# aurelienpierreeng/ansel

Measured on AMD Instinct MI355X. Metric: MPix/s full export pixelpipe (100 MP raw); % MI355X HBM roofline, higher is better.
Workload: dtype f32

## Files before the change

### ansel_amd/csrc/diffuse.hip

```cpp
#include "hip_common.h"

#include <type_traits>
#include "devmath.h"
#include "ieee_inrange.h"
#include "px_colorspaces.h"

#include <math.h>
#include <cstdlib>

namespace ansel
{
int bspline_launch_decompose(int devid, hipStream_t s, const float4 *in, float4 *hf, float4 *lf, int w, int h, int mult,
                             const unsigned *gate = nullptr);
int bspline_launch_decompose3(int devid, hipStream_t s, const void *in, bool in4, float *lf, int w, int h, int mult, unsigned *alpha_flag);
#ifdef ANSEL_HIP_MEASURING
int bspline_launch_decompose2(int devid, hipStream_t s, const float4 *in, float4 *low1, float4 *low2, int w, int h, int mult);
#endif
}
using namespace ansel;

namespace
{

#define DIFFUSE_MAX_SCALES 10
#define BSPLINE_SIGMA 1.0553651328015339f
#define PDE_KAPPA 0.25f

__device__ __forceinline__ float max_first(const float a, const float b) { return a > b ? a : b; }
__device__ __forceinline__ float max_zero(const float v) { return isfinite(v) ? max_first(v, 0.0f) : 0.0f; }
__device__ __forceinline__ int clampi(const int v, const int lo, const int hi) { return v < lo ? lo : (v > hi ? hi : v); }

__device__ __forceinline__ int walk_row(const int b, const int height, const int mult)
{
  if(height <= mult) return b < height ? b : -1;
  const int per_pass = (height + mult - 1) / mult;
  const int row = (b % per_pass) * mult + b / per_pass;
  return row < height ? row : -1;
}

struct pde_args
{
  int width, height, mult;
  float anisotropy[4];
  int kind[4];
  int same02, same13;
  float variance_threshold, regularization;
  float abcd[4], strength;
  int wskip;
  int post_lab;
  float post_m[3][4];
  int approx_div;
  int off;
  const unsigned *gate;
  int gate_sense;
};

#ifdef ANSEL_HIP_MEASURING
#define PDE_APPROX(a) ((a).approx_div != 0)
#define PDE_OFF(a, bit) (((a).off & (bit)) != 0)
#else
#define PDE_APPROX(a) false
#define PDE_OFF(a, bit) false
#endif
__device__ __forceinline__ float div_1ulp(const float x, const float y)
{
  const float r = __builtin_amdgcn_rcpf(y);
  const float q = x * r;
  return __builtin_fmaf(__builtin_fmaf(-y, q, x), r, q);
}

__device__ __forceinline__ float fast_expf(const float x)
{
  const float t = 1065353216.0f + x * 11401300.0f;
  int k = (t > -2147483648.0f && t < 2147483648.0f) ? (int)t : 0;
  k = k > 0 ? k : 0;
  return __int_as_float(k);
}

__device__ __forceinline__ float direction(float gx, float gy, float &cos2, float &sin2, float &cs, const bool approx = false)
{
  const float s2 = gx * gx + gy * gy;
// ... 286 lines not shown

#define PDE_RING 4
#define PDE_DMA_MAX_MULT 16
#if defined(__HIP_DEVICE_COMPILE__) && !defined(__gfx950__)
#error "pde_dma_planes(): LDS-DMA of 16 bytes per lane and its hazard padding are written for gfx950 only"
#endif
template <int NPL>
__device__ __forceinline__ void pde_dma_planes(const float4 *const p0, const float4 *const p1, const float4 *const p2, const unsigned voff,
                                               const unsigned d0, const unsigned d1, const unsigned d2)
{
  unsigned keep;
  if constexpr(NPL == 3)
    asm volatile("s_waitcnt lgkmcnt(0)\n\ts_nop 4\n\ts_mov_b32 %0, m0\n\t"
                 "s_mov_b32 m0, %5\n\ts_nop 0\n\tglobal_load_lds_dwordx4 %1, %2\n\t"
                 "s_mov_b32 m0, %6\n\ts_nop 0\n\tglobal_load_lds_dwordx4 %1, %3\n\t"
                 "s_mov_b32 m0, %7\n\ts_nop 0\n\tglobal_load_lds_dwordx4 %1, %4\n\t"
                 "s_mov_b32 m0, %0"
                 : "=&s"(keep)
                 : "v"(voff), "s"(p0), "s"(p1), "s"(p2), "s"(d0), "s"(d1), "s"(d2)
                 : "memory");
  else
    asm volatile("s_waitcnt lgkmcnt(0)\n\ts_nop 4\n\ts_mov_b32 %0, m0\n\t"
                 "s_mov_b32 m0, %4\n\ts_nop 0\n\tglobal_load_lds_dwordx4 %1, %2\n\t"
                 "s_mov_b32 m0, %5\n\ts_nop 0\n\tglobal_load_lds_dwordx4 %1, %3\n\t"
                 "s_mov_b32 m0, %0"
                 : "=&s"(keep)
                 : "v"(voff), "s"(p0), "s"(p2), "s"(d0), "s"(d2)
                 : "memory");
}
template <bool H0_4>
__device__ __forceinline__ void pde_dma_planes3(const void *const p0, const void *const p1, const void *const p2, const unsigned voff0,
                                                const unsigned voff, const unsigned d0, const unsigned d1, const unsigned d2)
{
  unsigned keep;
  if constexpr(H0_4)
    asm volatile("s_waitcnt lgkmcnt(0)\n\ts_nop 4\n\ts_mov_b32 %0, m0\n\t"
                 "s_mov_b32 m0, %6\n\ts_nop 0\n\tglobal_load_lds_dwordx4 %1, %3\n\t"
                 "s_mov_b32 m0, %7\n\ts_nop 0\n\tglobal_load_lds_dwordx3 %2, %4\n\t"
                 "s_mov_b32 m0, %8\n\ts_nop 0\n\tglobal_load_lds_dwordx3 %2, %5\n\t"
                 "s_mov_b32 m0, %0"
                 : "=&s"(keep)
                 : "v"(voff0), "v"(voff), "s"(p0), "s"(p1), "s"(p2), "s"(d0), "s"(d1), "s"(d2)
                 : "memory");
  else
    asm volatile("s_waitcnt lgkmcnt(0)\n\ts_nop 4\n\ts_mov_b32 %0, m0\n\t"
                 "s_mov_b32 m0, %5\n\ts_nop 0\n\tglobal_load_lds_dwordx3 %1, %2\n\t"
                 "s_mov_b32 m0, %6\n\ts_nop 0\n\tglobal_load_lds_dwordx3 %1, %3\n\t"
                 "s_mov_b32 m0, %7\n\ts_nop 0\n\tglobal_load_lds_dwordx3 %1, %4\n\t"
                 "s_mov_b32 m0, %0"
                 : "=&s"(keep)
                 : "v"(voff), "s"(p0), "s"(p1), "s"(p2), "s"(d0), "s"(d1), "s"(d2)
                 : "memory");
}
struct pde_px3
{
  float x, y, z;
};
template <bool HSUB, int MODE, bool DMA, int L3>
__device__ __forceinline__ void pde_strip_body(const float4 *__restrict__ hf, const float4 *__restrict__ hsub,
                                               const float4 *__restrict__ lf, float4 *__restrict__ out, const pde_args &a,
                                               const int final_pass, const unsigned char *__restrict__ mask, const int strip,
                                               const int strips_per_class)
{
  static_assert(L3 == 0 || (HSUB && DMA), "three-float planes: the low-pass chain's LDS-DMA form only");
  if(a.gate && ((*a.gate != 0u) == (a.gate_sense == 1))) return;
  extern __shared__ float4 r2s[];
  pde_px3 *const r2s3 = reinterpret_cast<pde_px3 *>(r2s);
  const int mult = a.mult;
  const int cls = blockIdx.y / strips_per_class, k0s = (blockIdx.y - cls * strips_per_class) * strip;
  const int n_cls = (a.height - cls + mult - 1) / mult;
  if(k0s >= n_cls) return;
  const int nrows = (strip < n_cls - k0s) ? strip : n_cls - k0s;
  const int r_first = cls + k0s * mult;
  const int tx = threadIdx.x, tw = 256 + 2 * mult;
  const int col = (int)blockIdx.x * 256 + tx;
  const bool live = col < a.width;
  const int cols[3] = { clampi(col - mult, 0, a.width - 1), clampi(col, 0, a.width - 1), clampi(col + mult, 0, a.width - 1) };
#define PDE_ROW(v) ((size_t)clampi(r_first + ((v) - 1) * mult, 0, a.height - 1) * a.width)
  float4 Hw[3][3], Lw[3][3];
  constexpr int NPL = HSUB ? 3 : 2;
  const int lane = tx & 63, zw = 64 + 2 * mult;
  float4 *const zone = r2s + PDE_RING * tw + (tx >> 6) * NPL * zw;
  float4 *const zone3 = reinterpret_cast<float4 *>(reinterpret_cast<char *>(r2s) + (size_t)PDE_RING * tw * 12) + (tx >> 6) * 3 * zw;
  using lds_f4_ptr = __attribute__((address_space(3))) float4 *;
  const unsigned zone_lds = !DMA ? 0u : (unsigned)__builtin_amdgcn_readfirstlane((int)(unsigned)(__UINTPTR_TYPE__)(lds_f4_ptr)(
                                           L3 ? zone3 : zone));
  const unsigned off_main = (unsigned)cols[0] * 16u, off_halo = (unsigned)clampi(col - mult + 64, 0, a.width - 1) * 16u;
  auto dma_row = [&](const int v) {
    const size_t y = PDE_ROW(v);
    if constexpr(L3 != 0)
    {
      const unsigned m3 = (unsigned)cols[0] * 12u, h3 = (unsigned)clampi(col - mult + 64, 0, a.width - 1) * 12u;
      const unsigned p0 = (unsigned)zw * 16u, p1 = 2u * p0;
      const void *const b0 = L3 == 2 ? (const void *)(hf + y) : (const void *)((const float *)hf + 3 * y);
      const void *const b1 = (const float *)hsub + 3 * y, *const b2 = (const float *)lf + 3 * y;
      pde_dma_planes3<L3 == 2>(b0, b1, b2, L3 == 2 ? off_main : m3, m3, zone_lds, zone_lds + p0, zone_lds + p1);
      if(lane < 2 * mult)
        pde_dma_planes3<L3 == 2>(b0, b1, b2, L3 == 2 ? off_halo : h3, h3, zone_lds + 1024u, zone_lds + p0 + 1024u, zone_lds + p1 + 1024u);
      return;
    }
    const unsigned pl = (unsigned)zw * 16u;
    pde_dma_planes<NPL>(hf + y, hsub + y, lf + y, off_main, zone_lds, zone_lds + pl, zone_lds + (NPL - 1) * pl);
    if(lane < 2 * mult)
      pde_dma_planes<NPL>(hf + y, hsub + y, lf + y, off_halo, zone_lds + 1024u, zone_lds + pl + 1024u, zone_lds + (NPL - 1) * pl + 1024u);
  };
  struct
  {
    float4 o;
    size_t idx;
    bool have;
  } pending;
  pending.have = false;
  auto store = [&](const size_t i, const float4 o) {
    if(final_pass) nt_store(out + i, o);
    else if constexpr(L3 != 0)
    {
      float *const p3 = (float *)out + 3 * i;
      p3[0] = o.x;
      p3[1] = o.y;
      p3[2] = o.z;
    }
    else out[i] = o;
  };
  auto fetch_row = [&](const int v, auto slot_tag) {
    constexpr int SL = decltype(slot_tag)::value;
    const size_t y = PDE_ROW(v);
    float4 c[3], low[3];
    if constexpr(DMA)
    {
      asm volatile("s_waitcnt vmcnt(0)" : : : "memory");
      if constexpr(L3 != 0)
      {
#pragma unroll
        for(int jj = 0; jj < 3; jj++)
        {
          const int x = lane + jj * mult;
          const float4 v0 = zone3[x], v1 = zone3[zw + x], v2 = zone3[2 * zw + x];
          c[jj] = make_float4(v0.x, v0.y, v0.z, 0.0f);
          low[jj] = make_float4(v1.x, v1.y, v1.z, 0.0f);
          Lw[SL][jj] = make_float4(v2.x, v2.y, v2.z, 0.0f);
        }
      }
      else
#pragma unroll
      for(int jj = 0; jj < 3; jj++)
      {
        c[jj] = zone[lane + jj * mult];
        if(HSUB) low[jj] = zone[zw + lane + jj * mult];
        Lw[SL][jj] = zone[(NPL - 1) * zw + lane + jj * mult];
      }
    }
    else if(PDE_OFF(a, 2) && v >= 2)
    {
#pragma unroll
      for(int jj = 0; jj < 3; jj++)
      {
        c[jj] = Hw[SL][jj];
        low[jj] = make_float4(0.f, 0.f, 0.f, 0.f);
      }
    }
    else
    {
#pragma unroll
      for(int jj = 0; jj < 3; jj++)
      {
        c[jj] = hf[y + cols[jj]];
        if(HSUB) low[jj] = hsub[y + cols[jj]];
        Lw[SL][jj] = lf[y + cols[jj]];
      }
    }
    __builtin_amdgcn_sched_barrier(0);
#pragma unroll
    for(int jj = 0; jj < 3; jj++)
      Hw[SL][jj] = HSUB ? make_float4(c[jj].x - low[jj].x, c[jj].y - low[jj].y, c[jj].z - low[jj].z, c[jj].w - low[jj].w) : c[jj];
    float4 *const ring = r2s + (v % PDE_RING) * tw;
    auto ratios = [&](const float4 h, const float4 l) {
      const bool blank = a.wskip && __builtin_amdgcn_ballot_w64((__float_as_uint(h.w) | __float_as_uint(l.w)) != 0) == 0ull;
      return ratio2_rgb(h, l, blank ? 0.0f : ratio2(h.w, l.w), PDE_APPROX(a));
    };
    if(PDE_OFF(a, 4)) return;
    if constexpr(L3 != 0)
    {
      pde_px3 *const ring3 = r2s3 + (v % PDE_RING) * tw;
      auto put = [&](const int x, const float4 h, const float4 l) {
        const float4 r = ratio2_rgb(h, l, 0.0f, PDE_APPROX(a));
        ring3[x] = { r.x, r.y, r.z };
      };
      put(tx + mult, Hw[SL][1], Lw[SL][1]);
      if(tx < mult) put(tx, Hw[SL][0], Lw[SL][0]);
      if(tx >= 256 - mult) put(tx + 2 * mult, Hw[SL][2], Lw[SL][2]);
      return;
    }
    ring[tx + mult] = ratios(Hw[SL][1], Lw[SL][1]);
    if(tx < mult) ring[tx] = ratios(Hw[SL][0], Lw[SL][0]);
    if(tx >= 256 - mult) ring[tx + 2 * mult] = ratios(Hw[SL][2], Lw[SL][2]);
  };
  auto row_step = [&](auto t_tag, const int kk) {
    constexpr int T = decltype(t_tag)::value, S0 = T, S1 = (T + 1) % 3, S2 = (T + 2) % 3;
    constexpr bool WIDE_READS = MODE >= 0 && !(((MODE % 3) | ((MODE / 9) % 3)) && (((MODE / 3) % 3) | ((MODE / 27) % 3)));
    fetch_row(kk + 2, std::integral_constant<int, S2>());
    if constexpr(DMA)
    {
      if(pending.have)
      {
        store(pending.idx, pending.o);
        pending.have = false;
      }
      if(kk + 1 < nrows) dma_row(kk + 3);
    }
    if(!PDE_OFF(a, 1)) __syncthreads();
    if(!live) return;
    const float4 H4[9] = { Hw[S0][0], Hw[S0][1], Hw[S0][2], Hw[S1][0], Hw[S1][1], Hw[S1][2], Hw[S2][0], Hw[S2][1], Hw[S2][2] };
    const float4 L4[9] = { Lw[S0][0], Lw[S0][1], Lw[S0][2], Lw[S1][0], Lw[S1][1], Lw[S1][2], Lw[S2][0], Lw[S2][1], Lw[S2][2] };
    const int row = r_first + kk * mult;
    const bool blank = L3 != 0 || alpha_is_blank(H4, L4);
    __builtin_amdgcn_sched_barrier(0);
    if(pending.have && !PDE_OFF(a, 8))
    {
      store(pending.idx, pending.o);
      pending.have = false;
    }
    __builtin_amdgcn_sched_barrier(0);
    float4 energy = make_float4(0.f, 0.f, 0.f, 0.f);
    if(PDE_OFF(a, 4)) energy = make_float4(0.5f, 0.5f, 0.5f, 0.5f);
    else if constexpr(L3 != 0)
#pragma unroll
    for(int ii = 0; ii < 3; ii++)
    {
      const pde_px3 *const ring = r2s3 + ((kk + ii) % PDE_RING) * tw + tx;
#pragma unroll
      for(int jj = 0; jj < 3; jj++)
      {
        const pde_px3 r = ring[jj * mult];
        energy.x += r.x;
        energy.y += r.y;
        energy.z += r.z;
      }
      if(!WIDE_READS || ii >= 1) asm volatile("" : "+v"(energy.x), "+v"(energy.y), "+v"(energy.z) : : "memory");
    }
    else
#pragma unroll
    for(int ii = 0; ii < 3; ii++)
    {
      const float4 *const ring = r2s + ((kk + ii) % PDE_RING) * tw + tx;
#pragma unroll
      for(int jj = 0; jj < 3; jj++)
      {
        const float4 r = ring[jj * mult];
        energy.x += r.x;
        energy.y += r.y;
        energy.z += r.z;
        if(!(blank && a.wskip)) energy.w += r.w;
      }
      if(!WIDE_READS || ii >= 1) asm volatile("" : "+v"(energy.x), "+v"(energy.y), "+v"(energy.z), "+v"(energy.w) : : "memory");
    }
    const size_t idx = (size_t)row * a.width + col;
    float4 o;
    if(L3 == 0 && mask && !mask[idx])
    {
      const float4 h = H4[4], l = L4[4];
      o = make_float4(max_zero(h.x + l.x), max_zero(h.y + l.y), max_zero(h.z + l.z), max_zero(h.w + l.w));
    }
    else if(PDE_OFF(a, 16))
      o = make_float4(H4[4].x + energy.x, L4[4].y + energy.y, H4[0].z + energy.z, L4[8].w);
    else
    {
      float H[9], L[9];
#pragma unroll
      for(int k = 0; k < 9; k++) { H[k] = H4[k].x; L[k] = L4[k].x; }
      o.x = pde_channel<MODE>(H, L, energy.x, a);
#pragma unroll
      for(int k = 0; k < 9; k++) { H[k] = H4[k].y; L[k] = L4[k].y; }
      o.y = pde_channel<MODE>(H, L, energy.y, a);
#pragma unroll
      for(int k = 0; k < 9; k++) { H[k] = H4[k].z; L[k] = L4[k].z; }
      o.z = pde_channel<MODE>(H, L, energy.z, a);
      if(blank)
        o.w = 0.0f;
      else
      {
#pragma unroll
        for(int k = 0; k < 9; k++) { H[k] = H4[k].w; L[k] = L4[k].w; }
        o.w = pde_channel<MODE>(H, L, energy.w, a);
      }
    }
    if(a.post_lab) o = px_rgb_to_lab(o, a.post_m);
    pending.o = o;
    pending.idx = idx;
    pending.have = true;
  };
  if constexpr(DMA) dma_row(0);
  fetch_row(0, std::integral_constant<int, 0>());
  if constexpr(DMA) dma_row(1);
  fetch_row(1, std::integral_constant<int, 1>());
  if constexpr(DMA) dma_row(2);
  for(int kk = 0; kk < nrows; kk += 3)
  {
    row_step(std::integral_constant<int, 0>(), kk);
    if(kk + 1 < nrows) row_step(std::integral_constant<int, 1>(), kk + 1);
    if(kk + 2 < nrows) row_step(std::integral_constant<int, 2>(), kk + 2);
  }
  if constexpr(DMA) asm volatile("s_waitcnt vmcnt(0)" : : : "memory");
  if(pending.have) store(pending.idx, pending.o);
#undef PDE_ROW
}

template <bool HSUB, int MODE, bool DMA = false>
__global__ __launch_bounds__(256, 3) void diffuse_pde_strip(const float4 *__restrict__ hf, const float4 *__restrict__ hsub,
                                                         const float4 *__restrict__ lf,
                                                         float4 *__restrict__ out, const pde_args a, const int final_pass,
                                                         const unsigned char *__restrict__ mask, const int strip,
                                                         const int strips_per_class)
{
  pde_strip_body<HSUB, MODE, DMA, 0>(hf, hsub, lf, out, a, final_pass, mask, strip, strips_per_class);
}
template <int MODE, bool H0_4>
__global__ __launch_bounds__(256, 3) void diffuse_pde_strip3(const float4 *__restrict__ hf, const float4 *__restrict__ hsub,
                                                          const float4 *__restrict__ lf, float4 *__restrict__ out, const pde_args a,
                                                          const int final_pass, const int strip, const int strips_per_class)
{
  pde_strip_body<true, MODE, true, H0_4 ? 2 : 1>(hf, hsub, lf, out, a, final_pass, nullptr, strip, strips_per_class);
}

__device__ __forceinline__ uint32_t splitmix32(const uint64_t seed)
{
  uint64_t result = (seed ^ (seed >> 33)) * 0x62a9d9ed799705f5ull;
  result = (result ^ (result >> 28)) * 0xcb24d0a5c88c35b3ull;
  return (uint32_t)(result >> 32);
}

__device__ __forceinline__ float xoshiro128plus(uint32_t state[4])
{
  const uint32_t result = state[0] + state[3];
  const uint32_t t = state[1] << 9;
  state[2] ^= state[0];
  state[3] ^= state[1];
  state[1] ^= state[2];
  state[0] ^= state[3];
  state[2] ^= t;
  state[3] = (state[3] << 11) | (state[3] >> 21);
  return (float)(result >> 8) * 0x1.0p-24f;
}

__device__ __forceinline__ float gaussian_noise(const float mu, const float sigma, const bool flip, uint32_t state[4])
{
  const float x1 = xoshiro128plus(state);
  const float u1 = x1 > 1.17549435e-38f ? x1 : 1.17549435e-38f;
  const float u2 = xoshiro128plus(state);
  const float angle = (float)(6.283185307179586 * (double)u2);
  const float radius = sqrtf(-2.0f * ansel_math::logf_exact(u1));
  const float noise = flip ? radius * ansel_math::cosf_exact(angle) : radius * ansel_math::sinf_exact(angle);
  return noise * sigma + mu;
}

__global__ __launch_bounds__(256) void diffuse_inpaint(const float4 *__restrict__ in, float4 *__restrict__ out,
                                                       unsigned char *__restrict__ mask, const float threshold,
                                                       const size_t npixels, const size_t width, const size_t first_pixel)
{
  const size_t p = (size_t)blockIdx.x * blockDim.x + threadIdx.x;
  if(p >= npixels) return;
  const float4 v = in[p];
  const bool m = v.x > threshold || v.y > threshold || v.z > threshold;
  mask[p] = m ? 1 : 0;
  float4 o = v;
  if(m)
  {
    const size_t k = 4 * (p + first_pixel);
    const uint32_t i = (uint32_t)(k / width);
    const uint32_t j = (uint32_t)(k - i);
    uint32_t state[4] = { splitmix32((uint32_t)(j + 1)), splitmix32((uint64_t)(uint32_t)(j + 1) * (uint32_t)(i + 3)),
                          splitmix32(1337), splitmix32(666) };
    xoshiro128plus(state);
    xoshiro128plus(state);
    xoshiro128plus(state);
    xoshiro128plus(state);
    const bool flip = (i % 2) || (j % 2);
    o.x = fabsf(gaussian_noise(v.x, v.x, flip, state));
    o.y = fabsf(gaussian_noise(v.y, v.y, flip, state));
    o.z = fabsf(gaussian_noise(v.z, v.z, flip, state));
    o.w = fabsf(gaussian_noise(v.w, v.w, flip, state));
  }
  out[p] = o;
}

inline float sqf(const float x) { return x * x; }

float sigma_at_step(const float sigma, const unsigned s)
{
  float acc = sigma;
  for(unsigned k = 1; k <= s; k++) acc = sqrtf(sqf(acc) + sqf(exp2f((float)k) * sigma));
  return acc;
}

unsigned steps_to_sigma(const float sigma_filter, const float sigma_final)
{
  unsigned s = 0;
  float radius = sigma_filter;
  while(radius < sigma_final)
  {
    ++s;
    radius = sqrtf(sqf(radius) + sqf((float)(1 << s) * sigma_filter));
  }
  return s + 1;
}

int scales_of(const dt_hip_piece_t *piece, const dt_hip_diffuse_data_t *d)
{
  const float zoom = (float)(d->iscale / piece->roi_in.scale);
  const float final_radius = (float)(d->radius + d->radius_center) * 2.0f / zoom;
  const int s = (int)steps_to_sigma(BSPLINE_SIGMA, final_radius);
  return s < 1 ? 1 : (s > DIFFUSE_MAX_SCALES ? DIFFUSE_MAX_SCALES : s);
}

}

namespace ansel
{
int diffuse_halo_rows(const dt_hip_piece_t *piece, const dt_hip_diffuse_data_t *d)
{
  if(!(d->iscale > 0.0f) || !(piece->roi_in.scale > 0.0)) return -1;
  const int scales = scales_of(piece, d);
  const int it_req = (int)ceilf((float)d->iterations);
  const int iterations = it_req > 1 ? it_req : 1;
  return iterations * 3 * ((1 << scales) - 1);
}
}

extern "C" {

int dt_hip_iop_diffuse_process(int devid, const dt_hip_piece_t *piece, const dt_hip_diffuse_data_t *d,
                               dt_hip_mem_t dev_in, dt_hip_mem_t dev_out)
{
  return diffuse_process_rows(devid, piece, d, 0, dev_in, dev_out);
}

}

namespace ansel
{
static void *g_diffuse_probe = nullptr;

static int diffuse_run(int devid, const dt_hip_piece_t *piece, const dt_hip_diffuse_data_t *d, int first_row, dt_hip_mem_t dev_in,
                       dt_hip_mem_t dev_out, const dt_hip_lab_data_t *post_lab);
int diffuse_process_rows(int devid, const dt_hip_piece_t *piece, const dt_hip_diffuse_data_t *d, int first_row,
                         dt_hip_mem_t dev_in, dt_hip_mem_t dev_out)
{
  return diffuse_run(devid, piece, d, first_row, dev_in, dev_out, nullptr);
}
int diffuse_process_post_lab(int devid, const dt_hip_piece_t *piece, const dt_hip_diffuse_data_t *d, dt_hip_mem_t dev_in,
                             dt_hip_mem_t dev_out, const dt_hip_lab_data_t *lab)
{
  if(!lab || measuring_env("ANSEL_HIP_PDE_PER_ROW")) return DT_HIP_INVALID_ARG;
  return diffuse_run(devid, piece, d, 0, dev_in, dev_out, lab);
}

struct diffuse_planes_t
{
  dev_buf_t hf[DIFFUSE_MAX_SCALES], lf[2], tmp[2];
  dev_buf_t mask;
  dev_buf_t inpainted;
  dev_buf_t alpha_flag;
};

struct diffuse_job_t
{
  int devid;
  hipStream_t st;
  const dt_hip_diffuse_data_t *d;
  const dt_hip_lab_data_t *post_lab;
  int w, h, scales, iterations;
  float zoom;
  bool lf_chain;
  bool per_row, no_dma;
  diffuse_planes_t p;
};

static int diffuse_alloc_planes(diffuse_job_t &j, const bool in_place, const bool three)
{
  diffuse_planes_t &p = j.p;
  const size_t plane = (size_t)j.w * j.h * sizeof(float4);
  bool ok = true;
  for(int s = 0; s < j.scales; s++) ok &= (bool)(p.hf[s] = dev_buf_t::alloc(j.devid, plane));
  for(int k = 0; k < ((j.lf_chain && !in_place) ? 1 : 2); k++) ok &= (bool)(p.lf[k] = dev_buf_t::alloc(j.devid, plane));
  for(int k = 0; k < 2 && k < j.iterations - 1; k++) ok &= (bool)(p.tmp[k] = dev_buf_t::alloc(j.devid, plane));
  if(ok && three) ok &= (bool)(p.alpha_flag = dev_buf_t::alloc(j.devid, sizeof(unsigned)));
  if(ok && j.d->threshold > 0.0f)
  {
    p.mask = dev_buf_t::alloc(j.devid, (size_t)j.w * j.h);
    if(!p.tmp[1]) p.tmp[1] = dev_buf_t::alloc(j.devid, plane);
    p.inpainted = dev_buf_t::borrow(p.tmp[1].base());
    ok = p.mask && p.inpainted;
  }
  return ok ? DT_HIP_SUCCESS : DT_HIP_SYSMEM_ALLOCATION;
}

static void pde_args_of_call(pde_args &a, const int w, const int h, const dt_hip_diffuse_data_t *d)
{
  memset(&a, 0, sizeof(a));
  a.width = w;
  a.height = h;
  a.wskip = measuring_env("ANSEL_HIP_PDE_NO_WSKIP") ? 0 : 1;
  const char *const approx_env = measuring_env("ANSEL_HIP_PDE_APPROX_DIV");
  a.approx_div = approx_env && atoi(approx_env) != 0;
  const char *const off_env = measuring_env("ANSEL_HIP_PDE_OFF");
  a.off = off_env ? atoi(off_env) : 0;
  const float user_aniso[4] = { d->anisotropy_first, d->anisotropy_second, d->anisotropy_third, d->anisotropy_fourth };
  for(int k = 0; k < 4; k++)
  {
    a.anisotropy[k] = sqf(user_aniso[k]);
    a.kind[k] = user_aniso[k] == 0.0f ? 0 : (user_aniso[k] > 0.0f ? 1 : 2);
  }
  a.same02 = a.kind[0] == a.kind[2] && a.anisotropy[0] == a.anisotropy[2];
  a.same13 = a.kind[1] == a.kind[3] && a.anisotropy[1] == a.anisotropy[3];
  a.variance_threshold = powf(10.0f, d->variance_threshold);
}

static void pde_args_of_scale(pde_args &a, const diffuse_job_t &j, const int s, const bool last_pass)
{
  const dt_hip_diffuse_data_t *const d = j.d;
  const float regularization = powf(10.0f, d->regularization) - 1.0f;
  const float speed[4] = { d->first, d->second, d->third, d->fourth };
  const float real_radius = sigma_at_step(BSPLINE_SIGMA, (unsigned)s) * j.zoom;
  a.regularization = regularization / 9.0f * sqf(real_radius);
  const float norm = expf(-sqf(real_radius - (float)d->radius_center) / sqf((float)d->radius));
  for(int k = 0; k < 4; k++) a.abcd[k] = speed[k] * PDE_KAPPA * norm;
  a.strength = d->sharpness * norm + 1.0f;
  a.mult = 1 << s;
  a.post_lab = 0;
  if(j.post_lab && last_pass)
  {
    a.post_lab = 1;
    memcpy(a.post_m, j.post_lab->matrix, sizeof(a.post_m));
  }
}

typedef void (*pde_strip_fn)(const float4 *, const float4 *, const float4 *, float4 *, pde_args, int, const unsigned char *, int, int);
typedef void (*pde_strip3_fn)(const float4 *, const float4 *, const float4 *, float4 *, pde_args, int, int, int);

template <int MD> static pde_strip_fn pde_strip_forms(const bool chain, const bool dma)
{
  if(dma) return diffuse_pde_strip<true, MD, true>;
  if(chain) return diffuse_pde_strip<true, MD>;
  return diffuse_pde_strip<false, MD>;
}
static pde_strip_fn pde_strip_kernel(const int mode, const bool chain, const bool dma)
{
  switch(mode)
  {
#define PDE_CASE(MD) \
  case MD: return pde_strip_forms<MD>(chain, dma);
    PDE_MODES(PDE_CASE)
#undef PDE_CASE
    default: return pde_strip_forms<-1>(chain, dma);
  }
}
static pde_strip3_fn pde_strip3_kernel(const int mode, const bool h0_4)
{
  if(mode == PDE_MODE_DEBLUR) return h0_4 ? diffuse_pde_strip3<PDE_MODE_DEBLUR, true> : diffuse_pde_strip3<PDE_MODE_DEBLUR, false>;
  return h0_4 ? diffuse_pde_strip3<PDE_MODE_ISOTROPIC, true> : diffuse_pde_strip3<PDE_MODE_ISOTROPIC, false>;
}

static void pde_strip_launch(const diffuse_job_t &j, const pde_args &a, const bool p3, const bool h0_4, const bool chain,
                             const bool dma, const float4 *h0, const float4 *h1, const float4 *cur, float4 *to,
                             const int final_pass)
{
  const int w = j.w, h = j.h;
  const int classes = h < a.mult ? h : a.mult, per_class = (h + a.mult - 1) / a.mult;
  const int gx = (w + 255) / 256;
  int longest = 32;
#ifdef ANSEL_HIP_MEASURING
  static const char *const strip_env = measuring_env("ANSEL_HIP_PDE_STRIP");
  if(strip_env) longest = atoi(strip_env);
#endif
  const int strip = strip_rows(gx, classes, per_class, longest);
  const int spc = (per_class + strip - 1) / strip;
  size_t ring = (size_t)PDE_RING * (256 + 2 * a.mult) * sizeof(float4);
#ifdef ANSEL_HIP_MEASURING
  static const char *const pad_env = measuring_env("ANSEL_HIP_PDE_LDS_PAD");
  if(pad_env) ring += (size_t)atoi(pad_env);
#endif
  static const bool generic = measuring_env("ANSEL_HIP_PDE_GENERIC") != nullptr;
  const int mode = generic ? -1 : pde_mode_of(a);
  const dim3 sgrid(gx, classes * spc);
  if(p3)
  {
    const size_t lds3 = (size_t)PDE_RING * (256 + 2 * a.mult) * 12 + (size_t)4 * 3 * (64 + 2 * a.mult) * 16;
    pde_strip3_kernel(mode, h0_4)<<<sgrid, 256, lds3, j.st>>>(h0, h1, cur, to, a, final_pass, strip, spc);
    return;
  }
  const size_t lds = dma ? ring + (size_t)4 * 3 * (64 + 2 * a.mult) * sizeof(float4) : ring;
  pde_strip_kernel(mode, chain, dma)<<<sgrid, 256, lds, j.st>>>(h0, h1, cur, to, a, final_pass, j.p.mask.as<unsigned char>(), strip, spc);
}

static int diffuse_iteration(const diffuse_job_t &j, pde_args &a, const bool p3, const bool first, const bool last,
                             const float4 *src, float4 *dst)
{
  const int w = j.w, h = j.h, scales = j.scales;
  float4 *hf[DIFFUSE_MAX_SCALES];
  for(int s = 0; s < DIFFUSE_MAX_SCALES; s++) hf[s] = j.p.hf[s].as<float4>();
  float4 *const lf[2] = { j.p.lf[0].as<float4>(), j.p.lf[1].as<float4>() };
  unsigned *const alpha_flag = j.p.alpha_flag.as<unsigned>();
  const unsigned char *const mask = j.p.mask.as<unsigned char>();
  int err = DT_HIP_SUCCESS;
  const float4 *level = src;
  float4 *residual = lf[0];
  const bool chain = j.lf_chain && (const float4 *)dst != src;
  for(int s = 0; s < scales && err == DT_HIP_SUCCESS; s++)
  {
#ifdef ANSEL_HIP_MEASURING
    static const bool pairs = measuring_env("ANSEL_HIP_BSPLINE_PAIRS") != nullptr;
    if(chain && pairs && s + 1 < scales && (s == 0 || s == 2))
    {
      err = bspline_launch_decompose2(j.devid, j.st, level, hf[s], hf[s + 1], w, h, 1 << s);
      s++;
      level = residual = hf[s];
      continue;
    }
#endif
    float4 *low = chain ? hf[s] : lf[s % 2];
    if(p3) err = bspline_launch_decompose3(j.devid, j.st, level, first && s == 0, (float *)low, w, h, 1 << s, alpha_flag);
    else err = bspline_launch_decompose(j.devid, j.st, level, chain ? nullptr : hf[s], low, w, h, 1 << s, alpha_flag);
    level = low;
    residual = low;
  }
  float4 *pp[2] = { residual == lf[1] ? lf[0] : lf[1], residual };
  const float4 *cur = residual;
  int count = 0;
  for(int s = scales - 1; s >= 0 && err == DT_HIP_SUCCESS; s--, count++)
  {
    pde_args_of_scale(a, j, s, s == 0 && last);
    float4 *to = (s == 0) ? dst : (chain ? (count % 2 == 0 ? lf[0] : hf[s + 1]) : pp[count % 2]);
    {
      launch_scope ls(j.devid, "diffuse_pde");
      if(a.mult <= PDE_SHARED_MULT && !j.per_row)
      {
        const float4 *const h0 = chain ? (s == 0 ? src : hf[s - 1]) : hf[s], *const h1 = chain ? hf[s] : nullptr;
        const bool dma = chain && a.mult <= PDE_DMA_MAX_MULT && !j.no_dma;
        pde_strip_launch(j, a, p3, first && s == 0, chain, dma, h0, h1, cur, to, p3 ? (s == 0 && last) : s == 0);
      }
      else
      {
        const int rows = (h <= a.mult) ? h : ((h + a.mult - 1) / a.mult) * a.mult;
        const dim3 grid(xcd_pad((w + 255) / 256), rows);
        if(a.mult <= PDE_SHARED_MULT)
          diffuse_pde<true><<<grid, 256, (size_t)3 * (256 + 2 * a.mult) * sizeof(float4), j.st>>>(hf[s], cur, to, a, s == 0, mask);
        else
          diffuse_pde<false><<<grid, 256, 0, j.st>>>(hf[s], cur, to, a, s == 0, mask);
      }
    }
    err = check_launch("diffuse_pde");
    cur = to;
  }
  return err;
}

static int diffuse_run(int devid, const dt_hip_piece_t *piece, const dt_hip_diffuse_data_t *d, int first_row, dt_hip_mem_t dev_in,
                       dt_hip_mem_t dev_out, const dt_hip_lab_data_t *post_lab)
{
  if(!valid_device(devid) || !piece || !d || !dev_in || !dev_out) return DT_HIP_INVALID_ARG;
  if(piece->channels != 4)
  {
    set_last_error("diffuse: needs a 4-channel float input");
    return DT_HIP_INVALID_ARG;
  }
  const int w = piece->roi_out.width, h = piece->roi_out.height;
  if(w <= 0 || h <= 0) return DT_HIP_SUCCESS;
  if(!(d->iscale > 0.0f) || !(piece->roi_in.scale > 0.0)) return DT_HIP_INVALID_ARG;
  static const bool per_row_pde = measuring_env("ANSEL_HIP_PDE_PER_ROW") != nullptr;
  static const bool hf_planes = measuring_env("ANSEL_HIP_DIFFUSE_HF_PLANES") != nullptr;
  static const bool no_dma = measuring_env("ANSEL_HIP_PDE_NO_DMA") != nullptr;
  const int it_req = (int)ceilf((float)d->iterations);
  diffuse_job_t j;
  j.devid = devid;
  j.st = stream_of(devid);
  j.d = d;
  j.post_lab = post_lab;
  j.w = w, j.h = h;
  j.scales = scales_of(piece, d);
  j.iterations = it_req > 1 ? it_req : 1;
  j.zoom = (float)(d->iscale / piece->roi_in.scale);
  j.lf_chain = !per_row_pde && !hf_planes && (1 << (j.scales - 1)) <= PDE_SHARED_MULT;
  j.per_row = per_row_pde, j.no_dma = no_dma;
  const int iterations = j.iterations;
  pde_args a;
  pde_args_of_call(a, w, h, d);

  const int mode0 = pde_mode_of(a);
  const bool in_place = iterations == 1 && dev_in == dev_out && !(d->threshold > 0.0f);
  const bool three = j.lf_chain && !no_dma && !(d->threshold > 0.0f) && (1 << (j.scales - 1)) <= PDE_DMA_MAX_MULT &&
                     !(iterations == 1 && dev_in == dev_out) && !measuring_env("ANSEL_HIP_PDE_GENERIC") &&
                     (mode0 == PDE_MODE_DEBLUR || mode0 == PDE_MODE_ISOTROPIC);
  int err = diffuse_alloc_planes(j, in_place, three);
  unsigned *const alpha_flag = j.p.alpha_flag.as<unsigned>();
  if(err == DT_HIP_SUCCESS && alpha_flag && hipMemsetAsync(alpha_flag, 0, sizeof(unsigned), j.st) != hipSuccess) err = DT_HIP_DEFAULT_ERROR;
  const float4 *src = (const float4 *)dev_in;
  if(err == DT_HIP_SUCCESS && j.p.mask)
  {
    const size_t np = (size_t)w * h;
    launch_scope ls(devid, "diffuse_inpaint");
    diffuse_inpaint<<<pixel_grid(np), 256, 0, j.st>>>(src, j.p.inpainted.as<float4>(), j.p.mask.as<unsigned char>(), d->threshold, np,
                                                      (size_t)w, (size_t)first_row * w);
    err = check_launch("diffuse_inpaint");
    src = j.p.inpainted.as<float4>();
  }
  for(int seq = alpha_flag ? 0 : 1; seq < 2 && err == DT_HIP_SUCCESS; seq++)
  {
    const bool p3 = seq == 0;
    a.gate = alpha_flag;
    a.gate_sense = p3 ? 1 : 2;
    if(alpha_flag) src = (const float4 *)dev_in;
    for(int it = 0; err == DT_HIP_SUCCESS && it < iterations; it++)
    {
      float4 *dst = (it == iterations - 1) ? (float4 *)dev_out : j.p.tmp[it % 2].as<float4>();
      err = diffuse_iteration(j, a, p3, it == 0, it == iterations - 1, src, dst);
      src = dst;
    }
  }
  if(alpha_flag)
  {
    if(g_diffuse_probe && err == DT_HIP_SUCCESS
       && hipMemcpyAsync(g_diffuse_probe, alpha_flag, sizeof(unsigned), hipMemcpyDeviceToDevice, j.st) != hipSuccess)
      err = DT_HIP_DEFAULT_ERROR;
  }
  else if(g_diffuse_probe && err == DT_HIP_SUCCESS && hipMemsetAsync(g_diffuse_probe, 0xff, sizeof(unsigned), j.st) != hipSuccess)
    err = DT_HIP_DEFAULT_ERROR;
  return err;
}

}

extern "C" {

int dt_hip_test_diffuse_probe(void *sink)
{
  ansel::g_diffuse_probe = sink;
  return DT_HIP_SUCCESS;
}

void dt_hip_iop_diffuse_tiling(const dt_hip_piece_t *piece, const dt_hip_diffuse_data_t *d, dt_hip_tiling_t *tiling)
{
  const int scales = scales_of(piece, d);
  tiling->factor = 6.0625f + scales;
  tiling->factor_cl = 6.0625f + scales;
  tiling->maxbuf = 1.0f;
  tiling->maxbuf_cl = 1.0f;
  tiling->overhead = 0;
  tiling->overlap = 1 << scales;
  tiling->xalign = 1;
  tiling->yalign = 1;
}

}
```

### ansel_amd/csrc/diffuse_bspline.hip

```cpp
#include "hip_common.h"

#include <cstdlib>

using namespace ansel;

namespace
{

__device__ __forceinline__ float max_first(const float a, const float b) { return a > b ? a : b; }
__device__ __forceinline__ int clampi(const int v, const int lo, const int hi) { return v < lo ? lo : (v > hi ? hi : v); }

__device__ __forceinline__ float tap5(const float a, const float b, const float c, const float d, const float e)
{
  const float s = 0.0625f * a + 0.25f * b + 0.375f * c + 0.25f * d + 0.0625f * e;
  return max_first(0.0f, s);
}
__device__ __forceinline__ float4 tap5(const float4 a, const float4 b, const float4 c, const float4 d, const float4 e)
{
  return make_float4(tap5(a.x, b.x, c.x, d.x, e.x), tap5(a.y, b.y, c.y, d.y, e.y), tap5(a.z, b.z, c.z, d.z, e.z),
                     tap5(a.w, b.w, c.w, d.w, e.w));
}

__device__ __forceinline__ int walk_row(const int b, const int height, const int mult)
{
  if(height <= mult) return b < height ? b : -1;
  const int per_pass = (height + mult - 1) / mult;
  const int row = (b % per_pass) * mult + b / per_pass;
  return row < height ? row : -1;
}

#ifdef ANSEL_HIP_MEASURING
__device__ __forceinline__ float4 vertical5(const float4 *__restrict__ in, const int width, const int height,
                                            const int row, const int col, const int mult, float4 *centre)
{
  const float4 a = in[(size_t)clampi(row - 2 * mult, 0, height - 1) * width + col];
  const float4 b = in[(size_t)clampi(row - mult, 0, height - 1) * width + col];
  const float4 c = in[(size_t)row * width + col];
  const float4 d = in[(size_t)clampi(row + mult, 0, height - 1) * width + col];
  const float4 e = in[(size_t)clampi(row + 2 * mult, 0, height - 1) * width + col];
  if(centre) *centre = c;
  return tap5(a, b, c, d, e);
}

template <int R, int T>
__global__ __launch_bounds__(256) void bspline_decompose(const float4 *__restrict__ in, float4 *__restrict__ hf,
                                                         float4 *__restrict__ lf, const int width, const int height,
                                                         const int mult, const int groups, const int gx)
{
  __shared__ float4 vert[(T + 4) * R + 2];
  const int bx = xcd_col();
  if(bx >= gx) return;
  const int row = walk_row(blockIdx.y, height, mult);
  if(row < 0) return;
  const int group = bx % groups, tile = bx / groups;
  const int r0 = group * R, k0 = tile * T;
  const int tid = threadIdx.x;
  const int r = tid % R, k = tid / R;
  const int col = r0 + r + (k0 + k) * mult;
  float4 centre = make_float4(0.f, 0.f, 0.f, 0.f);
  if(col < width) vert[(k + 2) * R + r] = vertical5(in, width, height, row, col, mult, &centre);
  if(tid < 4 * R)
  {
    const int hr = tid % R, hs = tid / R;
    const int hk = hs < 2 ? hs - 2 : T + hs - 2;
    const int hcol = r0 + hr + (k0 + hk) * mult;
    if(hcol >= 0 && hcol < width) vert[(hk + 2) * R + hr] = vertical5(in, width, height, row, hcol, mult, nullptr);
  }
  else if(tid == 4 * R)
    vert[(T + 4) * R] = vertical5(in, width, height, row, 0, mult, nullptr);
  else if(tid == 4 * R + 1)
    vert[(T + 4) * R + 1] = vertical5(in, width, height, row, width - 1, mult, nullptr);
  __syncthreads();
  if(col >= width) return;
  float4 t[5];
// ... 447 lines not shown
```

Baseline: 1625.

## Fuse coarsest B-spline decomposition into the final-scale PDE strip kernel

For the coarsest wavelet scale, the separate B-spline decompose pass is skipped. A new templated strip kernel variant computes the 5-tap vertical and horizontal low-pass inline from the previous level, using a rolling register window, an LDS staging area and LDS-DMA prefetch of the next row. It also derives the high-frequency plane and the ratio ring on the fly. This removes one full-image write and re-read of the low/high planes, at the cost of more LDS, extra barriers and duplicated halo filtering per block. The public process entry now enables this seam path, and a test hook can turn it off.

```diff
diff --git a/ansel_amd/csrc/diffuse.hip b/ansel_amd/csrc/diffuse.hip
--- a/ansel_amd/csrc/diffuse.hip
+++ b/ansel_amd/csrc/diffuse.hip
@@ -2,6 +2,7 @@
 
 #include <type_traits>
 #include "devmath.h"
+#include "diffuse_taps.h"
 #include "ieee_inrange.h"
 #include "px_colorspaces.h"
 
@@ -26,7 +27,8 @@
 #define BSPLINE_SIGMA 1.0553651328015339f
 #define PDE_KAPPA 0.25f
 
-__device__ __forceinline__ float max_first(const float a, const float b) { return a > b ? a : b; }
+using ansel_taps::max_first;
+using ansel_taps::tap5;
 __device__ __forceinline__ float max_zero(const float v) { return isfinite(v) ? max_first(v, 0.0f) : 0.0f; }
 __device__ __forceinline__ int clampi(const int v, const int lo, const int hi) { return v < lo ? lo : (v > hi ? hi : v); }
 
@@ -419,21 +421,37 @@
                  : "v"(voff), "s"(p0), "s"(p1), "s"(p2), "s"(d0), "s"(d1), "s"(d2)
                  : "memory");
 }
+__device__ __forceinline__ void pde_dma_row3(const void *const p, const unsigned voff, const unsigned dst)
+{
+  unsigned keep;
+  asm volatile("s_waitcnt lgkmcnt(0)\n\ts_nop 4\n\ts_mov_b32 %0, m0\n\t"
+               "s_mov_b32 m0, %3\n\ts_nop 0\n\tglobal_load_lds_dwordx3 %1, %2\n\t"
+               "s_mov_b32 m0, %0"
+               : "=&s"(keep)
+               : "v"(voff), "s"(p), "s"(dst)
+               : "memory");
+}
 struct pde_px3
 {
   float x, y, z;
 };
-template <bool HSUB, int MODE, bool DMA, int L3>
+__device__ __forceinline__ pde_px3 tap5(const pde_px3 a, const pde_px3 b, const pde_px3 c, const pde_px3 d, const pde_px3 e)
+{
+  return { tap5(a.x, b.x, c.x, d.x, e.x), tap5(a.y, b.y, c.y, d.y, e.y), tap5(a.z, b.z, c.z, d.z, e.z) };
+}
+template <bool HSUB, int MODE, bool DMA, int L3, int LOWIN = 0>
 __device__ __forceinline__ void pde_strip_body(const float4 *__restrict__ hf, const float4 *__restrict__ hsub,
                                                const float4 *__restrict__ lf, float4 *__restrict__ out, const pde_args &a,
                                                const int final_pass, const unsigned char *__restrict__ mask, const int strip,
                                                const int strips_per_class)
 {
   static_assert(L3 == 0 || (HSUB && DMA), "three-float planes: the low-pass chain's LDS-DMA form only");
+  static_assert(LOWIN == 0 || L3 == 1, "the coarsest seam: three-float planes only");
+  constexpr bool FETCH_DMA = DMA && LOWIN == 0;
   if(a.gate && ((*a.gate != 0u) == (a.gate_sense == 1))) return;
   extern __shared__ float4 r2s[];
   pde_px3 *const r2s3 = reinterpret_cast<pde_px3 *>(r2s);
-  const int mult = a.mult;
+  const int mult = LOWIN ? LOWIN : a.mult;
   const int cls = blockIdx.y / strips_per_class, k0s = (blockIdx.y - cls * strips_per_class) * strip;
   const int n_cls = (a.height - cls + mult - 1) / mult;
   if(k0s >= n_cls) return;
@@ -471,6 +489,24 @@
     if(lane < 2 * mult)
       pde_dma_planes<NPL>(hf + y, hsub + y, lf + y, off_halo, zone_lds + 1024u, zone_lds + pl + 1024u, zone_lds + (NPL - 1) * pl + 1024u);
   };
+  pde_px3 *const lw_v = r2s3 + PDE_RING * tw, *const lw_l = lw_v + 256 + 6 * mult, *const lw_h = lw_l + tw, *const lw_c = lw_h + tw;
+  const int seg = (int)blockIdx.x * 256;
+  int li = 0, ri = 0;
+  auto side_slots = [&]() {
+    int c = col;
+    asm volatile("" : "+v"(c));
+    li = clampi(c - mult, 0, a.width - 1) - seg + mult;
+    ri = clampi(c + mult, 0, a.width - 1) - seg + mult;
+  };
+  const pde_px3 z3 = { 0.f, 0.f, 0.f };
+  pde_px3 wa = z3, wb = z3, wc = z3, wd = z3, we = z3;
+  pde_px3 *const w2_0 = lw_c + 2 * mult;
+  char *const lw_n = reinterpret_cast<char *>(r2s) + (((size_t)((PDE_RING + 2) * tw + 256 + 38 * mult) * 12 + 15) & ~(size_t)15);
+  using lds_char_ptr = __attribute__((address_space(3))) char *;
+  const unsigned lw_n_lds = !LOWIN ? 0u : (unsigned)__builtin_amdgcn_readfirstlane((int)(unsigned)(__UINTPTR_TYPE__)(lds_char_ptr)(
+                                              lw_n + (tx >> 6) * 1024));
+  auto landed = [&](const int slot) { return *reinterpret_cast<const pde_px3 *>(lw_n + 16 * slot); };
+  auto wide = [](const pde_px3 p) { return make_float4(p.x, p.y, p.z, 0.0f); };
   struct
   {
     float4 o;
@@ -493,7 +529,87 @@
     constexpr int SL = decltype(slot_tag)::value;
     const size_t y = PDE_ROW(v);
     float4 c[3], low[3];
-    if constexpr(DMA)
+    if constexpr(LOWIN)
+    {
+      const pde_px3 *const in3 = reinterpret_cast<const pde_px3 *>(hf);
+      auto at = [&](const int row, const int x) { return in3[(size_t)clampi(row, 0, a.height - 1) * a.width + x]; };
+      int tq = tx;
+      asm volatile("" : "+v"(tq));
+      const int hx = tq - 64;
+      const bool second = hx >= 0 && hx < 6 * mult;
+      const int y2 = hx < 3 * mult ? hx : hx + 256, x2 = clampi(seg - 3 * mult + y2, 0, a.width - 1);
+      const int ex = tq - (256 - 2 * mult);
+      pde_px3 *const w2 = w2_0 + hx;
+      const int rc = r_first + (v - 1) * mult;
+      const int t0 = (v % 5) * 6 * mult, t5 = 30 * mult, t1 = t0 + 6 * mult < t5 ? t0 + 6 * mult : t0 - 24 * mult,
+                t2 = t0 + 12 * mult < t5 ? t0 + 12 * mult : t0 - 18 * mult, t3 = t0 + 18 * mult < t5 ? t0 + 18 * mult : t0 - 12 * mult,
+                t4 = t0 + 24 * mult < t5 ? t0 + 24 * mult : t0 - 6 * mult;
+      pde_px3 va = z3, vb = z3, vc = z3, vd = z3, ve = z3;
+      if(v == 0 || rc < 0 || rc >= a.height || (v == 1 && r_first < mult))
+      {
+        const int rr = clampi(rc, 0, a.height - 1);
+        wa = at(rr - 2 * mult, cols[1]);
+        wb = at(rr - mult, cols[1]);
+        wc = at(rr, cols[1]);
+        wd = at(rr + mult, cols[1]);
+        we = at(rr + 2 * mult, cols[1]);
+        if(second)
+        {
+          va = at(rr - 2 * mult, x2);
+          vb = at(rr - mult, x2);
+          vc = at(rr, x2);
+          vd = at(rr + mult, x2);
+          ve = at(rr + 2 * mult, x2);
+          w2[t0] = va, w2[t1] = vb, w2[t2] = vc, w2[t3] = vd, w2[t4] = ve;
+        }
+      }
+      else
+      {
+        asm volatile("s_waitcnt vmcnt(0)" : : : "memory");
+        wa = wb, wb = wc, wc = wd, wd = we, we = landed(tx);
+        if(second)
+        {
+          const pde_px3 vn = landed(256 + hx);
+          w2[t4] = vn;
+          va = w2[t0], vb = w2[t1], vc = w2[t2], vd = w2[t3], ve = vn;
+        }
+      }
+      lw_v[tx + 3 * mult] = tap5(wa, wb, wc, wd, we);
+      if(second)
+      {
+        lw_v[y2] = tap5(va, vb, vc, vd, ve);
+        if(hx >= 2 * mult && hx < 4 * mult) lw_c[hx - 2 * mult] = vc;
+      }
+      const pde_px3 *const next = in3 + (size_t)clampi(rc + 3 * mult, 0, a.height - 1) * a.width;
+      pde_dma_row3(next, (unsigned)cols[1] * 12u, lw_n_lds);
+      if(second) pde_dma_row3(next, (unsigned)x2 * 12u, lw_n_lds + 4096u - 1024u);
+      __syncthreads();
+      auto across = [&](const int x) {
+        pde_px3 t[5];
+#pragma unroll
+        for(int s = 0; s <= 4; s++) t[s] = lw_v[x + s * mult];
+        return tap5(t[0], t[1], t[2], t[3], t[4]);
+      };
+      pde_px3 *const ring3 = r2s3 + (v % PDE_RING) * tw;
+      auto leave = [&](const int slot, const pde_px3 cc, const pde_px3 l) {
+        const pde_px3 h = { cc.x - l.x, cc.y - l.y, cc.z - l.z };
+        lw_l[slot] = l;
+        lw_h[slot] = h;
+        const float4 r = ratio2_rgb(wide(h), wide(l), 0.0f, PDE_APPROX(a));
+        ring3[slot] = { r.x, r.y, r.z };
+        return h;
+      };
+      const pde_px3 l1 = across(tx + mult);
+      Lw[SL][1] = wide(l1);
+      Hw[SL][1] = wide(leave(tx + mult, wc, l1));
+      if(ex >= 0)
+      {
+        const int slot = ex < mult ? ex : 256 + ex;
+        leave(slot, lw_c[ex], across(slot));
+      }
+      return;
+    }
+    else if constexpr(DMA)
     {
       asm volatile("s_waitcnt vmcnt(0)" : : : "memory");
       if constexpr(L3 != 0)
@@ -562,6 +678,14 @@
     if(tx < mult) ring[tx] = ratios(Hw[SL][0], Lw[SL][0]);
     if(tx >= 256 - mult) ring[tx + 2 * mult] = ratios(Hw[SL][2], Lw[SL][2]);
   };
+  auto neighbours = [&](auto slot_tag) {
+    constexpr int SL = decltype(slot_tag)::value;
+    side_slots();
+    Lw[SL][0] = wide(lw_l[li]);
+    Lw[SL][2] = wide(lw_l[ri]);
+    Hw[SL][0] = wide(lw_h[li]);
+    Hw[SL][2] = wide(lw_h[ri]);
+  };
   auto row_step = [&](auto t_tag, const int kk) {
     constexpr int T = decltype(t_tag)::value, S0 = T, S1 = (T + 1) % 3, S2 = (T + 2) % 3;
     constexpr bool WIDE_READS = MODE >= 0 && !(((MODE % 3) | ((MODE / 9) % 3)) && (((MODE / 3) % 3) | ((MODE / 27) % 3)));
@@ -573,9 +697,11 @@
         store(pending.idx, pending.o);
         pending.have = false;
       }
-      if(kk + 1 < nrows) dma_row(kk + 3);
+      if constexpr(FETCH_DMA)
+        if(kk + 1 < nrows) dma_row(kk + 3);
     }
     if(!PDE_OFF(a, 1)) __syncthreads();
+    if constexpr(LOWIN) neighbours(std::integral_constant<int, S2>());
     if(!live) return;
     const float4 H4[9] = { Hw[S0][0], Hw[S0][1], Hw[S0][2], Hw[S1][0], Hw[S1][1], Hw[S1][2], Hw[S2][0], Hw[S2][1], Hw[S2][2] };
     const float4 L4[9] = { Lw[S0][0], Lw[S0][1], Lw[S0][2], Lw[S1][0], Lw[S1][1], Lw[S1][2], Lw[S2][0], Lw[S2][1], Lw[S2][2] };
@@ -594,11 +720,11 @@
 #pragma unroll
     for(int ii = 0; ii < 3; ii++)
     {
-      const pde_px3 *const ring = r2s3 + ((kk + ii) % PDE_RING) * tw + tx;
+      const pde_px3 *const ring = r2s3 + ((kk + ii) % PDE_RING) * tw + (LOWIN ? 0 : tx);
 #pragma unroll
       for(int jj = 0; jj < 3; jj++)
       {
-        const pde_px3 r = ring[jj * mult];
+        const pde_px3 r = ring[LOWIN ? (jj == 0 ? li : (jj == 1 ? tx + mult : ri)) : jj * mult];
         energy.x += r.x;
         energy.y += r.y;
         energy.z += r.z;
@@ -656,11 +782,21 @@
     pending.idx = idx;
     pending.have = true;
   };
-  if constexpr(DMA) dma_row(0);
+  if constexpr(FETCH_DMA) dma_row(0);
   fetch_row(0, std::integral_constant<int, 0>());
-  if constexpr(DMA) dma_row(1);
+  if constexpr(LOWIN)
+  {
+    __syncthreads();
+    neighbours(std::integral_constant<int, 0>());
+  }
+  if constexpr(FETCH_DMA) dma_row(1);
   fetch_row(1, std::integral_constant<int, 1>());
-  if constexpr(DMA) dma_row(2);
+  if constexpr(LOWIN)
+  {
+    __syncthreads();
+    neighbours(std::integral_constant<int, 1>());
+  }
+  if constexpr(FETCH_DMA) dma_row(2);
   for(int kk = 0; kk < nrows; kk += 3)
   {
     row_step(std::integral_constant<int, 0>(), kk);
@@ -687,6 +823,13 @@
                                                           const int final_pass, const int strip, const int strips_per_class)
 {
   pde_strip_body<true, MODE, true, H0_4 ? 2 : 1>(hf, hsub, lf, out, a, final_pass, nullptr, strip, strips_per_class);
+}
+template <int MODE, int MULT>
+__global__ __launch_bounds__(256, 4) void diffuse_pde_strip3_lowin(const float4 *__restrict__ hf, const float4 *__restrict__ hsub,
+                                                                const float4 *__restrict__ lf, float4 *__restrict__ out, const pde_args a,
+                                                                const int final_pass, const int strip, const int strips_per_class)
+{
+  pde_strip_body<true, MODE, true, 1, MULT>(hf, hsub, lf, out, a, final_pass, nullptr, strip, strips_per_class);
 }
 
 __device__ __forceinline__ uint32_t splitmix32(const uint64_t seed)
@@ -793,32 +936,24 @@
 }
 }
 
-extern "C" {
-
-int dt_hip_iop_diffuse_process(int devid, const dt_hip_piece_t *piece, const dt_hip_diffuse_data_t *d,
-                               dt_hip_mem_t dev_in, dt_hip_mem_t dev_out)
-{
-  return diffuse_process_rows(devid, piece, d, 0, dev_in, dev_out);
-}
-
-}
 
 namespace ansel
 {
 static void *g_diffuse_probe = nullptr;
+static int g_diffuse_seams_off = 0;
 
 static int diffuse_run(int devid, const dt_hip_piece_t *piece, const dt_hip_diffuse_data_t *d, int first_row, dt_hip_mem_t dev_in,
-                       dt_hip_mem_t dev_out, const dt_hip_lab_data_t *post_lab);
+                       dt_hip_mem_t dev_out, const dt_hip_lab_data_t *post_lab, bool seams);
 int diffuse_process_rows(int devid, const dt_hip_piece_t *piece, const dt_hip_diffuse_data_t *d, int first_row,
                          dt_hip_mem_t dev_in, dt_hip_mem_t dev_out)
 {
-  return diffuse_run(devid, piece, d, first_row, dev_in, dev_out, nullptr);
+  return diffuse_run(devid, piece, d, first_row, dev_in, dev_out, nullptr, false);
 }
 int diffuse_process_post_lab(int devid, const dt_hip_piece_t *piece, const dt_hip_diffuse_data_t *d, dt_hip_mem_t dev_in,
                              dt_hip_mem_t dev_out, const dt_hip_lab_data_t *lab)
 {
   if(!lab || measuring_env("ANSEL_HIP_PDE_PER_ROW")) return DT_HIP_INVALID_ARG;
-  return diffuse_run(devid, piece, d, 0, dev_in, dev_out, lab);
+  return diffuse_run(devid, piece, d, 0, dev_in, dev_out, lab, true);
 }
 
 struct diffuse_planes_t
@@ -838,6 +973,7 @@
   int w, h, scales, iterations;
   float zoom;
   bool lf_chain;
+  bool seams;
   bool per_row, no_dma;
   diffuse_planes_t p;
 };
@@ -921,13 +1057,24 @@
     default: return pde_strip_forms<-1>(chain, dma);
   }
 }
-static pde_strip3_fn pde_strip3_kernel(const int mode, const bool h0_4)
-{
+template <int MD> static pde_strip3_fn pde_strip3_lowin(const int mult)
+{
+  switch(mult)
+  {
+    case 2: return diffuse_pde_strip3_lowin<MD, 2>;
+    case 4: return diffuse_pde_strip3_lowin<MD, 4>;
+    case 8: return diffuse_pde_strip3_lowin<MD, 8>;
+    default: return diffuse_pde_strip3_lowin<MD, 16>;
+  }
+}
+static pde_strip3_fn pde_strip3_kernel(const int mode, const bool h0_4, const int lowin)
+{
+  if(lowin) return mode == PDE_MODE_DEBLUR ? pde_strip3_lowin<PDE_MODE_DEBLUR>(lowin) : pde_strip3_lowin<PDE_MODE_ISOTROPIC>(lowin);
   if(mode == PDE_MODE_DEBLUR) return h0_4 ? diffuse_pde_strip3<PDE_MODE_DEBLUR, true> : diffuse_pde_strip3<PDE_MODE_DEBLUR, false>;
   return h0_4 ? diffuse_pde_strip3<PDE_MODE_ISOTROPIC, true> : diffuse_pde_strip3<PDE_MODE_ISOTROPIC, false>;
 }
 
-static void pde_strip_launch(const diffuse_job_t &j, const pde_args &a, const bool p3, const bool h0_4, const bool chain,
+static void pde_strip_launch(const diffuse_job_t &j, const pde_args &a, const bool p3, const bool h0_4, const bool lowin, const bool chain,
                              const bool dma, const float4 *h0, const float4 *h1, const float4 *cur, float4 *to,
                              const int final_pass)
 {
@@ -951,8 +1098,9 @@
   const dim3 sgrid(gx, classes * spc);
   if(p3)
   {
-    const size_t lds3 = (size_t)PDE_RING * (256 + 2 * a.mult) * 12 + (size_t)4 * 3 * (64 + 2 * a.mult) * 16;
-    pde_strip3_kernel(mode, h0_4)<<<sgrid, 256, lds3, j.st>>>(h0, h1, cur, to, a, final_pass, strip, spc);
+    const size_t lds3 = lowin ? ((((size_t)((PDE_RING + 2) * (256 + 2 * a.mult) + 256 + 38 * a.mult) * 12 + 15) & ~(size_t)15) + (256 + 6 * a.mult) * 16)
+                              : (size_t)PDE_RING * (256 + 2 * a.mult) * 12 + (size_t)4 * 3 * (64 + 2 * a.mult) * 16;
+    pde_strip3_kernel(mode, h0_4, lowin ? a.mult : 0)<<<sgrid, 256, lds3, j.st>>>(h0, h1, cur, to, a, final_pass, strip, spc);
     return;
   }
   const size_t lds = dma ? ring + (size_t)4 * 3 * (64 + 2 * a.mult) * sizeof(float4) : ring;
@@ -972,11 +1120,12 @@
   const float4 *level = src;
   float4 *residual = lf[0];
   const bool chain = j.lf_chain && (const float4 *)dst != src;
-  for(int s = 0; s < scales && err == DT_HIP_SUCCESS; s++)
+  const bool lowin = p3 && chain && j.seams && scales >= 2 && !(g_diffuse_seams_off & 1);
+  for(int s = 0; s < (lowin ? scales - 1 : scales) && err == DT_HIP_SUCCESS; s++)
   {
 #ifdef ANSEL_HIP_MEASURING
     static const bool pairs = measuring_env("ANSEL_HIP_BSPLINE_PAIRS") != nullptr;
-    if(chain && pairs && s + 1 < scales && (s == 0 || s == 2))
+    if(chain && pairs && s + 1 < (lowin ? scales - 1 : scales) && (s == 0 || s == 2))
     {
       err = bspline_launch_decompose2(j.devid, j.st, level, hf[s], hf[s + 1], w, h, 1 << s);
       s++;
@@ -1003,7 +1152,7 @@
       {
         const float4 *const h0 = chain ? (s == 0 ? src : hf[s - 1]) : hf[s], *const h1 = chain ? hf[s] : nullptr;
         const bool dma = chain && a.mult <= PDE_DMA_MAX_MULT && !j.no_dma;
-        pde_strip_launch(j, a, p3, first && s == 0, chain, dma, h0, h1, cur, to, p3 ? (s == 0 && last) : s == 0);
+        pde_strip_launch(j, a, p3, first && s == 0, lowin && s == scales - 1, chain, dma, h0, h1, cur, to, p3 ? (s == 0 && last) : s == 0);
       }
       else
       {
@@ -1022,7 +1171,7 @@
 }
 
 static int diffuse_run(int devid, const dt_hip_piece_t *piece, const dt_hip_diffuse_data_t *d, int first_row, dt_hip_mem_t dev_in,
-                       dt_hip_mem_t dev_out, const dt_hip_lab_data_t *post_lab)
+                       dt_hip_mem_t dev_out, const dt_hip_lab_data_t *post_lab, const bool seams)
 {
   if(!valid_device(devid) || !piece || !d || !dev_in || !dev_out) return DT_HIP_INVALID_ARG;
   if(piece->channels != 4)
@@ -1048,6 +1197,7 @@
   j.zoom = (float)(d->iscale / piece->roi_in.scale);
   j.lf_chain = !per_row_pde && !hf_planes && (1 << (j.scales - 1)) <= PDE_SHARED_MULT;
   j.per_row = per_row_pde, j.no_dma = no_dma;
+  j.seams = seams;
   const int iterations = j.iterations;
   pde_args a;
   pde_args_of_call(a, w, h, d);
@@ -1098,9 +1248,21 @@
 
 extern "C" {
 
+int dt_hip_iop_diffuse_process(int devid, const dt_hip_piece_t *piece, const dt_hip_diffuse_data_t *d,
+                               dt_hip_mem_t dev_in, dt_hip_mem_t dev_out)
+{
+  return ansel::diffuse_run(devid, piece, d, 0, dev_in, dev_out, nullptr, true);
+}
+
 int dt_hip_test_diffuse_probe(void *sink)
 {
   ansel::g_diffuse_probe = sink;
+  return DT_HIP_SUCCESS;
+}
+
+int dt_hip_test_diffuse_seams(int mask)
+{
+  ansel::g_diffuse_seams_off = mask;
   return DT_HIP_SUCCESS;
 }
 
diff --git a/ansel_amd/csrc/diffuse_bspline.hip b/ansel_amd/csrc/diffuse_bspline.hip
--- a/ansel_amd/csrc/diffuse_bspline.hip
+++ b/ansel_amd/csrc/diffuse_bspline.hip
@@ -1,4 +1,5 @@
 #include "hip_common.h"
+#include "diffuse_taps.h"
 
 #include <cstdlib>
 
@@ -7,19 +8,9 @@
 namespace
 {
 
-__device__ __forceinline__ float max_first(const float a, const float b) { return a > b ? a : b; }
+using ansel_taps::max_first;
+using ansel_taps::tap5;
 __device__ __forceinline__ int clampi(const int v, const int lo, const int hi) { return v < lo ? lo : (v > hi ? hi : v); }
-
-__device__ __forceinline__ float tap5(const float a, const float b, const float c, const float d, const float e)
-{
-  const float s = 0.0625f * a + 0.25f * b + 0.375f * c + 0.25f * d + 0.0625f * e;
-  return max_first(0.0f, s);
-}
-__device__ __forceinline__ float4 tap5(const float4 a, const float4 b, const float4 c, const float4 d, const float4 e)
-{
-  return make_float4(tap5(a.x, b.x, c.x, d.x, e.x), tap5(a.y, b.y, c.y, d.y, e.y), tap5(a.z, b.z, c.z, d.z, e.z),
-                     tap5(a.w, b.w, c.w, d.w, e.w));
-}
 
 __device__ __forceinline__ int walk_row(const int b, const int height, const int mult)
 {
diff --git a/ansel_amd/csrc/diffuse_taps.h b/ansel_amd/csrc/diffuse_taps.h
--- /dev/null
+++ b/ansel_amd/csrc/diffuse_taps.h
@@ -0,0 +1,21 @@
+#pragma once
+
+#include <hip/hip_runtime.h>
+
+namespace ansel_taps
+{
+
+__device__ __forceinline__ float max_first(const float a, const float b) { return a > b ? a : b; }
+
+__device__ __forceinline__ float tap5(const float a, const float b, const float c, const float d, const float e)
+{
+  const float s = 0.0625f * a + 0.25f * b + 0.375f * c + 0.25f * d + 0.0625f * e;
+  return max_first(0.0f, s);
+}
+__device__ __forceinline__ float4 tap5(const float4 a, const float4 b, const float4 c, const float4 d, const float4 e)
+{
+  return make_float4(tap5(a.x, b.x, c.x, d.x, e.x), tap5(a.y, b.y, c.y, d.y, e.y), tap5(a.z, b.z, c.z, d.z, e.z),
+                     tap5(a.w, b.w, c.w, d.w, e.w));
+}
+
+}
```

After: 1632 (median of 6 runs). No clear change (+0.4%).
